# JuliaGraphics/Hikari.jl

Measured on AMD Instinct MI355X. Metric: Mrays/s, higher is better.
Workload: dtype f32

## Files before the change

### hikari.jl_amd/csrc/hk_ctx.cpp

```cpp
#include "hk_host.h"

thread_local std::string g_err;
SlabCache g_slabs;

namespace hk {
static thread_local const Knobs* tl_knobs = nullptr;
const char* knob(const char* name) {
    if (!tl_knobs) return nullptr;
    auto it = tl_knobs->kv.find(name);
    return it == tl_knobs->kv.end() ? nullptr : it->second.c_str();
}
static const char* const KNOB_NAMES[] = {
    "HK_BATCH_PATHS_M", "HK_BVH_LEAF", "HK_BVH_BINS", "HK_QNODES", "HK_DEBUG_ALLOC", "HK_DELTA_ADVANCE", "HK_DYNAMIC_SEGMENTS", "HK_GREY", "HK_GREY_COMPACT", "HK_GREY_FLAT", "HK_MAX_PATHS_M",
    "HK_MID_LISTS", "HK_MID_PASS_PATHS_M", "HK_NODE_CACHE", "HK_NVDB_DENSE_MB", "HK_OVERLAP", "HK_PIPELINE", "HK_PIPELINE_AFTER", "HK_PIPELINE_MAX_PATHS_M", "HK_PRESELECT",
    "HK_SELECT_MIN_IDLE", "HK_SHADOW_FEED_ROUNDS", "HK_SHADOW_TRACK_BATCH", "HK_SMALL_PASS", "HK_SMALL_PASS_WAVES", "HK_SOBOL_LO_GB", "HK_SOBOL_TABLE_ONLY",
    "HK_STATE_CACHE_GB", "HK_STATE_SLAB", "HK_TICKET_SHARE", "HK_TRACK_ADVANCE", "HK_TRACK_EXTRA_ADVANCE", "HK_TRACK_MIN_PENDING", "HK_TRACK_POOL", "HK_TRACK_REFILL_IDLE",
    "HK_WALK_POOL", "HK_WALK_REFILL_IDLE", "HK_WALK_SPLIT", "HK_WAVES_PER_CU", "HK_READBACK_PIN", "HK_DEFER_EXTERNAL", "HK_SELECT_POOL", "HK_SMALL_PASS_FUSED", "HK_SMALL_PASS_MERGED", "HK_OCC_SCALE", "HK_ESCAPED_UNROLL", "HK_SHADOW_FINAL", "HK_TRI_PACK", "HK_LEAN_RECORDS", "HK_VIEW_CACHE", "HK_MAJORANT_BLOCK_VOXELS", "HK_BVH_BUILD_SMALL", "HK_SHADE_LEAN", "HK_SHADE_PRESCAN", "HK_SHADE_PREFETCH"};
static bool known_knob(const char* name) {
    for (const char* k : KNOB_NAMES)
        if (std::strcmp(k, name) == 0) return true;
    return false;
}
}
KnobScope::KnobScope(const hk::Knobs* k) : prev(hk::tl_knobs) { hk::tl_knobs = k; }
KnobScope::~KnobScope() { hk::tl_knobs = prev; }

void quiesce(hk_ctx* c) {
    if (!c) return;
    (void)hipStreamSynchronize(c->stream);
    if (c->aux) (void)hipStreamSynchronize(c->aux);
    for (auto& l : c->lanes)
        if (l.stream) (void)hipStreamSynchronize(l.stream);
}
int join_lanes(hk_ctx* c) {
    if (!c) return HK_OK;
    if (int e = flush_pending(c)) return e;
    if (!c->lanes_dirty) return HK_OK;
    for (auto& l : c->lanes)
        if (l.done) HIP_TRY(hipStreamWaitEvent(c->stream, l.done, 0));
    c->lanes_dirty = false;
// ... 326 lines not shown
```

### hikari.jl_amd/csrc/hk_edit_host.h

```cpp
#pragma once
#include <algorithm>
#include <cmath>
#include <cstddef>
#include <cstring>
#include <vector>

#if defined(__HIPCC__)
#define HK_EDIT_HD __host__ __device__
#else
#define HK_EDIT_HD
#endif

HK_EDIT_HD inline double hk_box_area(const float lo[3], const float hi[3]) {
    if (!(lo[0] <= hi[0]) || !(lo[1] <= hi[1]) || !(lo[2] <= hi[2])) return 0.0;
    const double dx = (double)hi[0] - (double)lo[0], dy = (double)hi[1] - (double)lo[1], dz = (double)hi[2] - (double)lo[2];
    return 2.0 * ((dx * dy + dx * dz) + dy * dz);
}
HK_EDIT_HD inline double hk_node_cost(const float lo[2][3], const float hi[2][3], int c0, int c1) {
    const double w0 = c0 >= 0 ? 1.0 : (double)(((~c0) & 7) + 1), w1 = c1 >= 0 ? 1.0 : (double)(((~c1) & 7) + 1);
    return hk_box_area(lo[0], hi[0]) * w0 + hk_box_area(lo[1], hi[1]) * w1;
}
HK_EDIT_HD inline double hk_root_area(const float lo[2][3], const float hi[2][3]) {
    float l[3] = {INFINITY, INFINITY, INFINITY}, h[3] = {-INFINITY, -INFINITY, -INFINITY};
    for (int c = 0; c < 2; ++c) {
        if (!(lo[c][0] <= hi[c][0]) || !(lo[c][1] <= hi[c][1]) || !(lo[c][2] <= hi[c][2])) continue;
        for (int k = 0; k < 3; ++k) l[k] = lo[c][k] < l[k] ? lo[c][k] : l[k], h[k] = h[k] < hi[c][k] ? hi[c][k] : h[k];
    }
    return hk_box_area(l, h);
}

namespace hk {

template <class Material>
inline int materials_have_kind(const Material* m, size_t n, int kind) {
    for (size_t i = 0; i < n; ++i)
        if (m[i].kind == kind) return 1;
    return 0;
}
inline int single_material_kind(unsigned kinds_mask, int has_mix, int max_kinds) {
    if (has_mix || kinds_mask == 0u || (kinds_mask & (kinds_mask - 1u)) != 0u) return -1;
    int k = 0;
    while (!((kinds_mask >> k) & 1u)) ++k;
    return k < max_kinds ? k : -1;
}

inline bool stage_positions(const float* src, int first, int n, float* dst, int block, std::vector<float>& fresh) {
    fresh.clear();
    const int b0 = block > 0 ? first / block : 0;
    if (block > 0) {
        const int nb = (first + n - 1) / block - b0 + 1;
        fresh.resize(6 * (size_t)nb);
        for (int b = 0; b < nb; ++b)
            for (int k = 0; k < 3; ++k) fresh[6 * (size_t)b + k] = INFINITY, fresh[6 * (size_t)b + 3 + k] = -INFINITY;
    }
    bool finite = true;
    for (int i = 0; i < n; ++i) {
        const float* p = src + 9 * (size_t)i;
        std::memcpy(dst + 9 * (size_t)i, p, 36);
        for (int v = 0; v < 9; ++v) finite = finite && std::isfinite(p[v]);
        if (block > 0) {
            float* bb = fresh.data() + 6 * (size_t)((first + i) / block - b0);
            for (int v = 0; v < 9; ++v) {
                bb[v % 3] = std::min(bb[v % 3], p[v]);
                bb[3 + v % 3] = std::max(bb[3 + v % 3], p[v]);
            }
        }
    }
// ... 40 lines not shown
```

### hikari.jl_amd/csrc/hk_kernels.hip

```cpp
#include <hip/hip_runtime.h>
#include <type_traits>
#include <cstdlib>
#include <cstdio>

#include "hikari_mi355x.h"
#include "hk_device.h"
#include "hk_edit_host.h"
#include "hk_bvh_decide.h"

using namespace hkd;

namespace {

__device__ __forceinline__ int lane_id() { return (int)(threadIdx.x & 63); }

struct WaveQ {
    uint32_t* base;
    int count;
};
__device__ __forceinline__ int global_wave() {
    const int w = (int)(threadIdx.x >> 6), b = (int)blockIdx.x;
    if (blockDim.x == 1024 && (gridDim.x & 7) == 0) return ((((b >> 3) * 4 + (w >> 2)) * 8 + (b & 7)) << 2) + (w & 3);
    if (blockDim.x == 512 && (gridDim.x & 7) == 0) return ((((b >> 3) * 2 + (w >> 2)) * 8 + (b & 7)) << 2) + (w & 3);
    return b * (int)(blockDim.x >> 6) + w;
// ... 753 lines not shown
    HK_DBG_DECL
    HK_FOR_EACH_SEGMENT_FROM(gw, st, src) {
    const DPathGen g = gen_at(st, depth);
    const uint32_t seg = (uint32_t)gw * (uint32_t)st.wave_cap;
    const int n = *count_ptr(st, depth, Q_RAY, gw);
    WaveQ q_escaped = wq_open(st.escaped_q, st, gw);
    static_assert(!(SINGLE && MIX), "a scene with a MixMaterial is not a single-kind scene");
    int kind_count[HK_MAX_KINDS];
#pragma unroll
    for (int k = 0; k < HK_MAX_KINDS; ++k) kind_count[k] = 0;
    int one_count = 0;
    int cursor = 0;
    int state = LR_EMPTY;
    uint32_t slot = 0;
    LaneRay r;
    r.cur = r.pend = DONE;
    for (;;) {
        const unsigned long long run_m = __ballot(state == LR_ACTIVE && r.cur != DONE);
        if (run_m == 0ull || (64 - __popcll(run_m) >= MIN_IDLE && cursor < n)) {
            HK_DBG(8, state == LR_ACTIVE && r.cur == DONE);
            int kind = -1;
            uint32_t eflag = 0u;
            if (state == LR_ACTIVE && r.cur == DONE) {
                if (r.best.prim < 0)
                    kind = -2;
                else {
                    ++n_hits;
                    const DTriMeta hm = sc.meta[r.best.prim];
                    eflag = hm.arealight > 0 ? HK_MATQ_EMISSIVE : 0u;
                    int mat = sc.mis[hm.mi].material;
                    if (MIX && sc.materials[mat].kind == HK_MAT_MIX) {
                        float w = 1.0f - r.best.u - r.best.v;
                        mat = resolve_mix_material(sc, mat, r.o + r.d * r.best.t, -r.d, uv_at(sc, r.best.prim, w, r.best.u, r.best.v));
                    }
                    kind = SINGLE ? sc.single_kind : sc.materials[mat].kind;
                    if (MIX && kind == HK_MAT_MIX) kind = HK_MAT_FALLBACK;
                    stream_st(&st.hit[slot], make_float4(r.best.t, __int_as_float(r.best.prim), r.best.u, r.best.v));
                    stream_st(reinterpret_cast<uint32_t*>(st.mat_id) + slot, (uint32_t)(mat | (hm.arealight > 0 ? HK_MAT_EMISSIVE_BIT : 0)));
                }
                state = LR_EMPTY;
            }
            wq_push(q_escaped, slot, kind == -2);
            unsigned long long pending = __ballot(kind >= 0);
            if (SINGLE) {
                if (kind >= 0) stream_st(&st.mat_q[((size_t)sc.single_kind * st.n_waves + gw) * st.wave_cap + one_count + __popcll(pending & lt_mask)], slot | eflag);
                one_count += __popcll(pending);
                pending = 0ull;
            }
            while (pending) {
// ... 1545 lines not shown
    st4(&st.L[pmeta.y], ld4(&st.L[pmeta.y]) + fin);
}

template <int KIND>
struct ShadeWaves {
    static constexpr int value = (KIND == HK_MAT_COATED_DIFFUSE || KIND == HK_MAT_COATED_DIFFUSE_TRANSMISSION) ? 1 : (KIND == HK_MAT_MATTE ? HK_SHADE_WAVES_MATTE : HK_SHADE_WAVES);
};
#ifndef HK_SHADE_MIN_WAVES
#define HK_SHADE_MIN_WAVES 1
#endif
#define HK_SHADE_STASH 16
struct ShadeStage {
    uint32_t* entry;
    float4* hit;
    float4* ray_d;
    uint32_t* meta;
};
__device__ __forceinline__ void lds_fetch4(const uint32_t* src, uint32_t* lds_wave_base) {
    __builtin_amdgcn_global_load_lds((const __attribute__((address_space(1))) void*)src, (__attribute__((address_space(3))) void*)lds_wave_base, 4, 0, 0);
}
__device__ __forceinline__ void lds_fetch16(const float4* src, float4* lds_wave_base) {
    __builtin_amdgcn_global_load_lds((const __attribute__((address_space(1))) void*)src, (__attribute__((address_space(3))) void*)lds_wave_base, 16, 0, 0);
}
template <int KIND, bool SIMPLE, bool FT, bool PRE, bool LEAN = false>
__device__ __forceinline__ void shade_body(const DPathState& st, const DScene& sc, const DTables& T, const DFrame& fr, const DSobol& sob, int depth, int first_kind, DStats* stats, const SegTickets& src,
                                           uint32_t* __restrict__ elist,
                                           float* stash = nullptr,
                                           ShadeStage stage = ShadeStage{}) {
    static_assert(!LEAN || (KIND == HK_MAT_MATTE && HK_LAMBDA_BY_SLOT), "the lean body is Matte's");
    const int lane = lane_id();
    unsigned n_vertices = 0, n_lnodes = 0;
    unsigned nv_wave = 0;
    unsigned* const nl_stash = LEAN ? reinterpret_cast<unsigned*>(stash) + (HK_SHADE_STASH - 1) * 256 + threadIdx.x : nullptr;
    auto nl_flush = [&]() {
        if constexpr (LEAN) {
            if (n_lnodes) *nl_stash += n_lnodes;
            n_lnodes = 0;
        }
    };
    if constexpr (LEAN) *nl_stash = 0u;
    auto uni = [](int v) { return LEAN ? __builtin_amdgcn_readfirstlane(v) : v; };
    HK_FOR_EACH_SEGMENT_FROM(gw_v, st, src) {
    const int gw = uni(gw_v);
    const uint32_t* __restrict__ queue = st.mat_q + ((size_t)KIND * st.n_waves + gw) * st.wave_cap;
    const int n = uni(*count_ptr(st, depth, Q_MAT0 + KIND, gw));
    const DPathGen g = gen_at(st, depth), gn = st.gen[(depth + 1) & 1];
    const size_t seg = (size_t)gw * st.wave_cap;
    const bool ones = depth == 0 && fr.implicit_ones;
    WavePos q_shadow{0}, q_next{0};
    if (!first_kind) {
        q_shadow.count = uni(*count_ptr(st, depth, Q_SHADOW, gw));
        q_next.count = uni(*count_ptr(st, depth + 1, Q_RAY, gw));
    }
    int n_emit = 0;
    auto emit_pass = [&](int take) {
        __builtin_amdgcn_fence(__ATOMIC_SEQ_CST, "wavefront");
        if (lane < take) shade_emission<KIND == HK_MAT_MATTE, SIMPLE, LEAN>(st, g, ones, sc, T, elist[lane], n_lnodes, depth, seg);
        nl_flush();
        const int rest = n_emit - take;
        const uint32_t moved = lane < rest ? elist[64 + lane] : 0u;
        __builtin_amdgcn_fence(__ATOMIC_SEQ_CST, "wavefront");
        if (lane < rest) elist[lane] = moved;
        n_emit = rest;
    };
    const bool prescan = uni(st.shade_prescan) != 0;
    if (prescan) {
        for (int base = 0; base < n || n_emit > 0; base += 64) {
            if (base < n) {
                const int i = base + lane;
                const uint32_t cand = i < n ? queue[i] & ~HK_MATQ_EMISSIVE : 0u;
                const bool em = i < n && (st.mat_id[cand] & HK_MAT_EMISSIVE_BIT) != 0;
                const unsigned long long m = __ballot(em);
                if (em) elist[n_emit + __popcll(m & ((1ull << lane) - 1ull))] = cand;
                n_emit += __popcll(m);
                if (n_emit < 64 && base + 64 < n) continue;
            }
            emit_pass(n_emit < 64 ? n_emit : 64);
        }
    }
    const bool prefetch = LEAN && stage.entry != nullptr;
    const int wave0 = LEAN ? __builtin_amdgcn_readfirstlane((int)(threadIdx.x & ~63u)) : 0;
    if constexpr (LEAN) {
        if (prefetch && 64 + lane < n) lds_fetch4(&queue[64 + lane], stage.entry + 256 + wave0);
    }
    for (int base = 0; base < n; base += 64) {
        int i = base + lane;
        bool active = i < n;
        if constexpr (LEAN) {
            if (prefetch && i + 128 < n) lds_fetch4(&queue[i + 128], stage.entry + ((base >> 6) & 1) * 256 + wave0);
        }
        const bool staged = prefetch && base > 0;
        uint32_t slot = active ? queue[i] : 0u;
        {
            const bool em = !prescan && (slot & HK_MATQ_EMISSIVE) != 0u;
            slot &= ~HK_MATQ_EMISSIVE;
            const unsigned long long m = __ballot(em);
            if (m != 0ull) {
                if (em) elist[n_emit + __popcll(m & ((1ull << lane) - 1ull))] = slot;
                n_emit += __popcll(m);
                if (n_emit >= 64) emit_pass(64);
            }
        }
        bool push_shadow = false, push_ray = false;
        float4 H = make_float4(0, 0, 0, 0);
        Surface sf;
        v3 wo = mk3(0, 0, 1);
        DTriMeta meta{0u, 0u, 0u};
        S4 lambda = s4(0.0f), beta = s4(0.0f), r_u = s4(0.0f), kd_matte = s4(0.0f);
        uint32_t fl = 0, pslot = 0;
        int pdepth = 0, medium = -1;
        bool any_non_specular = false;
        SobolCtx sctx;
        using W = std::conditional_t<LEAN, float, S4>;
        auto stash_at = [&]() {
            int i = (int)threadIdx.x;
            asm volatile("" : "+v"(i));
            return stash + i;
        };
        const int base_dim = 6 + 7 * depth;
        float4 shO = make_float4(0, 0, 0, 0), shD = shO;
        S4 shLd = s4(0.0f);
        W shRu{}, shRl{};
        if constexpr (LEAN) nv_wave += (unsigned)(n - base < 64 ? n - base : 64);
        if (active) {
            if constexpr (!LEAN) ++n_vertices;
            float4 D;
            uint32_t meta_w = 0;
            if (LEAN && staged) {
                asm volatile("s_waitcnt vmcnt(0)" ::: "memory");
                const int t = (int)threadIdx.x;
                H = stage.hit[t], D = stage.ray_d[t], meta_w = stage.meta[t];
            } else {
                H = stream_ld(&st.hit[slot]);
                D = stream_ld(&g.ray_d[slot]);
                if constexpr (LEAN) meta_w = reinterpret_cast<const uint32_t*>(g.meta)[slot];
            }
            float4 O = ld_ray_o(st, g, slot, depth, seg);
            v3 ro = mk3(O.x, O.y, O.z), rd = mk3(D.x, D.y, D.z);
            float t_hit = H.x;
            int prim = __float_as_int(H.y);
            sf = surface_at(sc, prim, H.z, H.w, ro, rd, t_hit);
            wo = -rd;
            meta = tri_meta(sc, prim);
            if constexpr (LEAN) {
                pslot = meta_w & 0x3fffffffu;
                pdepth = depth;
                any_non_specular = (meta_w >> 31) != 0u;
            } else {
                const uint2 pmeta = ld_meta(st, g, slot, depth);
                fl = pmeta.x;
                pslot = pmeta.y;
// ... 52 lines not shown
                    asm volatile("" : "+v"(b2));
                    Surface s2 = surface_at(sc, prim, b2, H.w, ro, rd, t_hit);
                    sink = s2.pi.x + s2.n.y + s2.ns.z + s2.uv.x + s2.area;
                }
                if (HK_ABLATE == 6) {
                    v3 w2 = wo;
                    asm volatile("" : "+v"(w2.x), "+v"(w2.y), "+v"(w2.z));
                    float p2;
                    S4 f2 = eval_matte_kd(kd_matte, w2, sf.n, sf.ns, p2);
                    BSDFSample s2 = sample_matte_kd(sc, sc.materials[st.mat_id[slot] & ~HK_MAT_EMISSIVE_BIT], kd_matte, w2, sf.ns, TexCtx(sf.uv, meta.prim_index, H.z, H.w), mk2(H.z, H.w));
                    sink = f2.x + f2.w + p2 + s2.pdf + s2.wi.x + s2.f.y;
                }
                asm volatile("" : : "v"(sink));
            }
#endif

            if constexpr (LEAN) {
                float* sp = stash + threadIdx.x;
                sp[0 * 256] = sf.n.x, sp[1 * 256] = sf.n.y, sp[2 * 256] = sf.n.z;
                sp[3 * 256] = wo.x, sp[4 * 256] = wo.y, sp[5 * 256] = wo.z;
                sp[6 * 256] = kd_matte.x, sp[7 * 256] = kd_matte.y, sp[8 * 256] = kd_matte.z, sp[9 * 256] = kd_matte.w;
                sp[10 * 256] = beta.x, sp[11 * 256] = beta.y, sp[12 * 256] = beta.z, sp[13 * 256] = beta.w;
                sp[14 * 256] = __uint_as_float(meta_w);
                if (prefetch && i + 64 < n) {
                    asm volatile("s_waitcnt vmcnt(0)" ::: "memory");
                    const uint32_t ns = stage.entry[(((base >> 6) + 1) & 1) * 256 + (int)threadIdx.x] & ~HK_MATQ_EMISSIVE;
                    lds_fetch16(&st.hit[ns], stage.hit + wave0);
                    lds_fetch16(&g.ray_d[ns], stage.ray_d + wave0);
                    lds_fetch4(reinterpret_cast<const uint32_t*>(g.meta) + ns, stage.meta + wave0);
                }
            }
            if (sc.n_lights > 0) {
                const DMaterial& mat = sc.materials[st.mat_id[slot] & ~HK_MAT_EMISSIVE_BIT];
                float light_pmf;
                int light_idx;
                if constexpr (PRE) {
                    const uint2 pre = st.sel_light[slot];
                    light_idx = (int)pre.x;
                    light_pmf = __uint_as_float(pre.y);
                } else {
                    float light_select = sobol_1d<FT>(sctx, base_dim + 1);
                    light_idx = bvh_sample_light(sc, sf.pi, sf.ns, light_select, light_pmf, n_lnodes);
                }
                if (light_idx >= 1 && light_idx <= sc.n_lights && light_pmf > 0.0f) {
                    const DLight& sel = sc.lights[light_idx - 1];
                    v2 u_light = mk2(0.0f, 0.0f);
                    if (sel.kind >= HK_LIGHT_AMBIENT) u_light = sobol_2d<FT>(sctx, base_dim + 3);
// ... 139 lines not shown
                if (st.compact) nD.w = nrl.x;
                stream_st(&gn.ray_d[pn], nD);
                stream_st(&gn.beta[pn], nb);
                st_ru_rl(gn, pn, r_u, nrl, st.compact != 0);
                st_lambda(gn, pn, lambda);
                st_meta(st, gn, pn, nflags, pslot);
            }
        }
    }
    if (n_emit > 0) emit_pass(n_emit);
    if (lane == 0) {
        *count_ptr(st, depth, Q_SHADOW, gw) = q_shadow.count;
        *count_ptr(st, depth + 1, Q_RAY, gw) = q_next.count;
    }
    }
    if constexpr (LEAN) {
        n_vertices = lane == 0 ? nv_wave : 0u;
        n_lnodes = *nl_stash;
    }
    stats += global_wave();
    wave_add(&stats->vertices, n_vertices);
    wave_add(&stats->light_nodes, n_lnodes);
}
template <int KIND, bool SIMPLE = false, bool FT = false, bool PRE = false, bool LEAN = false>
__global__ void __attribute__((amdgpu_flat_work_group_size(256, 256), amdgpu_waves_per_eu(LEAN ? (FT ? HK_SHADE_WAVES_LEAN : HK_SHADE_WAVES_LEAN_HASH) : ShadeWaves<KIND>::value))) k_shade(DPathState st, DScene sc, DTables T, DFrame fr, DSobol sob, int depth, int first_kind, DStats* stats) {
    __shared__ uint32_t emit_list[4 * 128];
    SegTickets src = seg_open(st, ticket_ptr(st, depth, TK_SHADE0 + KIND), st.dynamic_segments != 0, depth, Q_MAT0 + KIND);
    if constexpr (LEAN) {
        src.pos = __builtin_amdgcn_readfirstlane(src.pos), src.k0 = __builtin_amdgcn_readfirstlane(src.k0);
        __shared__ float stash[HK_SHADE_STASH * 256];
        __shared__ uint32_t stage_entry[2 * 256];
        __shared__ float4 stage_hit[256];
        __shared__ float4 stage_ray_d[256];
        __shared__ uint32_t stage_meta[256];
        ShadeStage stage{};
        if (st.shade_prefetch) stage.entry = stage_entry, stage.hit = stage_hit, stage.ray_d = stage_ray_d, stage.meta = stage_meta;
        shade_body<KIND, SIMPLE, FT, PRE, true>(st, sc, T, fr, sob, depth, first_kind, stats, src, emit_list + (threadIdx.x >> 6) * 128, stash, stage);
    } else
        shade_body<KIND, SIMPLE, FT, PRE>(st, sc, T, fr, sob, depth, first_kind, stats, src, emit_list + (threadIdx.x >> 6) * 128);
}

template <class W> HKD W wone();
template <> HKD float wone<float>() { return 1.0f; }
template <> HKD S4 wone<S4>() { return s4(1.0f); }
HKD S4 wide(S4 v) { return v; }
HKD S4 wide(float v) { return s4(v); }
HKD bool is_black(float v) { return v == 0.0f; }
template <bool COMPACT>
HKD void shadow_contribute(const DPathState& st, uint32_t rec, S4 T_ray, S4 tr_u, S4 tr_l) {
    if (is_black(T_ray)) return;
    S4 w_u, w_l;
    ld_shadow_weights<COMPACT>(st, rec, w_u, w_l);
    S4 mis = w_u * tr_u + w_l * tr_l;
    float den = average(mis);
    if (den > 1e-10f) {
        S4 fin = ld4(&st.sh_Ld[rec]) * T_ray / den;
        if (!is_black(fin)) {
            const uint32_t pslot = st.sh_slot[rec];
            st4(&st.L[pslot], ld4(&st.L[pslot]) + fin);
        }
// ... 2180 lines not shown
```

### hikari.jl_amd/csrc/hk_launch_impl.h

```cpp
#pragma once
#include "hk_launch.h"

namespace hk {

template <bool V>
using bool_c = std::bool_constant<V>;
template <int V>
using int_c = std::integral_constant<int, V>;
template <class F>
static void with_bool(bool b, F&& f) {
    if (b) f(bool_c<true>{});
    else f(bool_c<false>{});
}
template <int V0, int... Vs, class F>
static void with_int(int v, F&& f) {
    if constexpr (sizeof...(Vs) == 0) f(int_c<V0>{});
    else if (v == V0) f(int_c<V0>{});
    else with_int<Vs...>(v, f);
}

#ifndef HK_OCC_SCALE_DEFAULT
#define HK_OCC_SCALE_DEFAULT 1.0f
#endif
static inline int grid_for(int n, int block, int cap) {
// ... 73 lines not shown
#endif
#ifndef HK_SHADOW_BLOCK16
#define HK_SHADOW_BLOCK16 768
#endif
#ifndef HK_SHADOW_NC32
#define HK_SHADOW_NC32 0
#endif
#ifndef HK_TRACE_SINGLE_KIND
#define HK_TRACE_SINGLE_KIND 1
#endif
#ifndef HK_TRACE_NC32
#define HK_TRACE_NC32 128
#endif
template <int B16, int NC16, int NC32, class F>
static void lean_dispatch(const DScene& sc, const DFrame& fr, F&& launch) {
    with_bool(fr.count_nodes != 0, [&](auto COUNT) {
        with_bool(node_cache_on(), [&](auto CACHE) {
            constexpr bool cache = decltype(CACHE)::value;
            if (sc.bvh_depth <= 16) launch(COUNT, int_c<16>{}, int_c<cache ? B16 : HK_TRACE_BLOCK>{}, int_c<cache ? NC16 : 0>{}, bool_c<false>{});
            else with_bool(sc.qnodes != nullptr, [&](auto QN) { launch(COUNT, int_c<HK_LDS_STACK>{}, int_c<HK_TRACE_BLOCK>{}, int_c<cache ? NC32 : 0>{}, QN); });
        });
    });
}
void launch_trace(hipStream_t s, int n_cu, const DPathState& st, const DScene& sc, const DTables& T, const DFrame& fr, int depth, DStats* stats) {
    if (lean_scene(sc)) {
        const int flush = sc.has_mix ? 0 : (HK_TRACE_SINGLE_KIND && sc.single_kind >= 0 ? 2 : 1);
        lean_dispatch<1024, 1536, HK_TRACE_NC32>(sc, fr, [&](auto COUNT, auto STACK, auto BLOCK, auto NC, auto QN) {
            constexpr int block = decltype(BLOCK)::value;
            constexpr bool count = decltype(COUNT)::value;
            with_int<2, 1, 0>(flush, [&](auto FLUSH) {
                constexpr int f = count ? 0 : decltype(FLUSH)::value;
                launch_resident<k_trace_lean<count, decltype(STACK)::value, block, decltype(NC)::value, decltype(QN)::value, f == 0, f == 2>>(s, n_cu, st, block, 8, sc, depth, stats);
            });
        });
        return;
    }
    with_bool(fr.count_nodes != 0, [&](auto COUNT) { launch_resident<k_trace<decltype(COUNT)::value>>(s, n_cu, st, HK_TRACE_BLOCK, 8, sc, T, fr, depth, stats); });
}
template <bool C, int MM>
static void launch_walk_split(hipStream_t s, int n_cu, const DPathState& st, const DScene& sc, const DFrame& fr, int depth, DStats* stats) {
    const int cb = clamp_blocks(cached_blocks<k_walk_cast<C, MM, 16>>(HK_TRACE_BLOCK, n_cu, 8), st);
    const int tb = clamp_blocks(cached_blocks<k_walk_track<MM>>(256, n_cu, 8), st);
    for (int round = 0; round < HK_WALK_ROUNDS; ++round) {
        hipLaunchKernelGGL((k_walk_cast<C, MM, 16>), dim3(cb), dim3(HK_TRACE_BLOCK), 0, s, st, sc, depth, round, stats, sc.media);
        hipLaunchKernelGGL((k_walk_track<MM>), dim3(tb), dim3(256), 0, s, st, sc, depth, round, fr.walk_tune, stats, sc.media);
    }
}
bool grey_compact_ok(const DScene& sc) {
    if (!knob_on("HK_GREY_COMPACT")) return false;
// ... 86 lines not shown
    hipLaunchKernelGGL(k_detect_camera_medium, dim3(1), dim3(64), 0, s, st, sc, x, y, z, stats);
}
void launch_escaped(hipStream_t s, int n_cu, const DPathState& st, const DScene& sc, const DTables& T, const DFrame& fr, int depth) {
    with_bool(knob_int("HK_ESCAPED_UNROLL", 1) != 2, [&](auto ONE) { launch_resident<k_escaped<decltype(ONE)::value ? 1 : 2>>(s, n_cu, st, 256, 8, sc, T, depth, fr.implicit_ones); });
}
bool preselect_lights(const DScene& sc, const DPathState& st) {
    return sc.n_media == 0 && sc.num_bvh_lights >= HK_PRESELECT_MIN && st.sel_light != nullptr && knob_on("HK_PRESELECT");
}
void launch_light_select(hipStream_t s, int n_cu, const DPathState& st, const DScene& sc, const DTables& T, const DFrame& fr, const DSobol& sob, int depth, uint32_t kinds_mask, DStats* stats) {
    const int min_idle = knob_int_in("HK_SELECT_MIN_IDLE", 1, 64, HK_SELECT_MIN_IDLE);
    const bool pool = knob_on("HK_SELECT_POOL");
    with_bool(sobol_tables_cover(sob, depth), [&](auto FT) {
        constexpr bool ft = decltype(FT)::value;
        if (pool) launch_resident<k_light_select_pool<ft>>(s, n_cu, st, HK_SELECT_BLOCK, 8, sc, T, fr, sob, depth, kinds_mask, stats);
        else launch_resident<k_light_select<ft>>(s, n_cu, st, 256, 8, sc, T, fr, sob, depth, kinds_mask, min_idle, stats);
    });
}
void launch_shade(hipStream_t s, int n_cu, int kind, const DPathState& st, const DScene& sc, const DTables& T, const DFrame& fr, const DSobol& sob, int depth, int first_kind, DStats* stats) {
    auto shade = [&](auto KIND, auto SIMPLE, auto FT, auto PRE) {
        launch_resident<k_shade<decltype(KIND)::value, decltype(SIMPLE)::value, decltype(FT)::value, decltype(PRE)::value>>(s, n_cu, st, 256, 8, sc, T, fr, sob, depth, first_kind, stats);
    };
    const bool ft = sobol_tables_cover(sob, depth);
    if (kind == HK_MAT_MATTE && sc.simple_lights && lean_scene(sc) && st.compact && st.meta32 && st.sh_final && !preselect_lights(sc, st) && knob_on("HK_SHADE_LEAN")) {
        with_bool(ft, [&](auto FT) { launch_resident<k_shade<HK_MAT_MATTE, true, decltype(FT)::value, false, true>>(s, n_cu, st, 256, 8, sc, T, fr, sob, depth, first_kind, stats); });
        return;
    }
    const bool light_kind = kind == HK_MAT_MATTE || kind == HK_MAT_MIRROR || kind == HK_MAT_GLASS || kind == HK_MAT_CONDUCTOR;
    if (light_kind && preselect_lights(sc, st))
        with_int<HK_MAT_MATTE, HK_MAT_MIRROR, HK_MAT_GLASS, HK_MAT_CONDUCTOR>(kind, [&](auto KIND) { with_bool(ft, [&](auto FT) { shade(KIND, bool_c<false>{}, FT, bool_c<true>{}); }); });
    else if (kind == HK_MAT_MATTE && sc.simple_lights)
        with_bool(ft, [&](auto FT) { shade(int_c<HK_MAT_MATTE>{}, bool_c<true>{}, FT, bool_c<false>{}); });
    else if (light_kind && ft)
        with_int<HK_MAT_MATTE, HK_MAT_MIRROR, HK_MAT_GLASS, HK_MAT_CONDUCTOR>(kind, [&](auto KIND) { shade(KIND, bool_c<false>{}, bool_c<true>{}, bool_c<false>{}); });
    else
        with_int<HK_MAT_MATTE, HK_MAT_MIRROR, HK_MAT_GLASS, HK_MAT_CONDUCTOR, HK_MAT_COATED_DIFFUSE, HK_MAT_THIN_DIELECTRIC, HK_MAT_DIFFUSE_TRANSMISSION, HK_MAT_COATED_DIFFUSE_TRANSMISSION,
                 HK_MAT_COATED_CONDUCTOR, HK_MAT_FALLBACK>(kind, [&](auto KIND) { shade(KIND, bool_c<false>{}, bool_c<false>{}, bool_c<false>{}); });
}
#ifndef HK_SMALL_PASS_NC
#define HK_SMALL_PASS_NC 1536
#endif
static int small_pass_class(const DScene& sc, uint32_t kinds_mask) {
    const int mode = knob_int("HK_SMALL_PASS_FUSED", 2);
    if (mode == 0) return 0;
    if (!(lean_scene(sc) && sc.bvh_depth <= HK_LDS_STACK && node_cache_on())) return 0;
    if (kinds_mask == (1u << HK_MAT_MATTE) && sc.simple_lights && !sc.has_escape_lights && sc.bvh_depth <= 16 && sc.num_bvh_lights < HK_PRESELECT_MIN) return 1;
    const uint32_t light_kinds = (1u << HK_MAT_MATTE) | (1u << HK_MAT_MIRROR) | (1u << HK_MAT_GLASS) | (1u << HK_MAT_CONDUCTOR);
    return (mode >= 2 && kinds_mask != 0 && (kinds_mask & ~light_kinds) == 0) ? 2 : 0;
// ... 166 lines not shown
```

### hikari.jl_amd/csrc/hk_render.cpp

```cpp
#include "hk_host.h"

namespace {
float gaussian_1d(float x, float sigma) { return std::exp(-(x * x) / (2.0f * (sigma * sigma))); }
float mitchell_1d(float x, float B, float C) {
    x = std::fabs(x);
    if (x <= 1.0f) return ((12.0f - 9.0f * B - 6.0f * C) * (x * x * x) + (-18.0f + 12.0f * B + 6.0f * C) * (x * x) + (6.0f - 2.0f * B)) / 6.0f;
    if (x <= 2.0f) return ((-B - 6.0f * C) * (x * x * x) + (6.0f * B + 30.0f * C) * (x * x) + (-12.0f * B - 48.0f * C) * x + (8.0f * B + 24.0f * C)) / 6.0f;
    return 0.0f;
}
float sinc1(float x) {
    x = std::fabs(x);
    if (x < 1e-5f) return 1.0f;
    x *= 3.14159265358979323846f;
    return std::sin(x) / x;
}
float wsinc(float x, float r, float tau) {
    x = std::fabs(x);
    if (x > r) return 0.0f;
    return sinc1(x) * sinc1(x / tau);
}
float filter_eval(const hk_integrator_params& p, float ex, float ey, float x, float y) {
    float rx = p.filter_radius[0], ry = p.filter_radius[1];
    switch (p.filter_type) {
        case HK_FILTER_BOX: return (std::fabs(x) <= rx && std::fabs(y) <= ry) ? 1.0f : 0.0f;
// ... 192 lines not shown
}
int ensure_state(hk_integrator* I, int capacity, const PassTraits& t, hipStream_t users) {
    const bool media = t.media, open_scene = t.open_scene, small_scene = t.small_scene, grey_compact = t.grey_compact, fusable = t.fusable, lean = t.lean;
    const int n_cu = I->ctx->n_cu;
    long mid_paths = 48L << 20;
    if (const char* e = hk::knob("HK_MID_PASS_PATHS_M")) mid_paths = std::atol(e) >= 0 ? std::atol(e) << 20 : mid_paths;
    const bool mid = !media && !open_scene && small_scene && (long)capacity <= mid_paths;
    I->mid_pass = mid;
    const long cap_per_cu = media ? 96 : ((open_scene || mid) ? 48 : 192);
    long W_want = ((long)(capacity + 63) / 64) / 16;
    if (W_want < 4L * n_cu) W_want = 4L * n_cu;
    if (W_want > cap_per_cu * n_cu) W_want = cap_per_cu * n_cu;
    I->ctx->waves_per_cu = hk::knob_int_in("HK_WAVES_PER_CU", 1, INT_MAX, 0);
    if (I->ctx->waves_per_cu > 0) W_want = (long)I->ctx->waves_per_cu * n_cu;
    W_want = (W_want + 3) / 4 * 4;
    I->st.dynamic_segments = (media || (!open_scene && !mid)) ? 1 : 0;
    I->st.dynamic_segments = hk::knob_int("HK_DYNAMIC_SEGMENTS", I->st.dynamic_segments) ? 1 : 0;
    I->st.compact = media ? (grey_compact ? 1 : 0) : 1;
    I->st.sh_final = (lean && hk::knob_on("HK_SHADOW_FINAL")) ? 1 : 0;
    I->st.meta32 = (lean && hk::knob_on("HK_LEAN_RECORDS")) ? 1 : 0;
    I->st.const_origin = 0;
    I->st.shade_prescan = hk::knob_int("HK_SHADE_PRESCAN", 0) != 0 ? 1 : 0;
    I->st.shade_prefetch = hk::knob_on("HK_SHADE_PREFETCH") ? 1 : 0;
    I->st.ticket_share = hk::knob_int("HK_TICKET_SHARE", 1) ? 1 : 0;
    {
        const bool small_on = hk::knob_on("HK_SMALL_PASS");
        const bool small = W_want <= 4L * n_cu && small_on && hk::knob("HK_DYNAMIC_SEGMENTS") == nullptr;
        I->st.small_pass = small ? 1 : 0;
        if (mid && I->st.dynamic_segments == 0 && small_on && !hk::knob_int("HK_MID_LISTS", 0))
            I->st.small_pass = 1;
        if (small) {
            I->st.dynamic_segments = 0;
            const int w = hk::knob_int_in("HK_SMALL_PASS_WAVES", 1, INT_MAX, 0);
            long per_cu = w > 0 ? w : (users ? (media ? 4 : 8) : (((open_scene && !media) || fusable) ? 8 : 16));
            const long chunks = ((long)capacity + 63) / 64;
            while (per_cu > 4 && per_cu * n_cu > chunks) per_cu /= 2;
            if (I->ctx->waves_per_cu <= 0) W_want = (per_cu * n_cu + 3) / 4 * 4;
        }
    }
    const bool want_split = media && hk::walk_split_mode();
    const bool want_cam = !media && !users && hk::knob_on("HK_VIEW_CACHE");
    if (I->st_capacity >= capacity && I->st_depth >= I->p.max_depth && I->st.n_waves == (int)W_want && I->st_media == (media ? 1 : 0) && (!want_split || I->st.wq_a != nullptr) &&
        (!want_cam || I->cam_gen.ray_d != nullptr || I->cam_unfit))
        return HK_OK;
    I->view_key.clear();
    if (users) HIP_TRY(hipStreamSynchronize(users));
// ... 500 lines not shown
```

### hikari.jl_amd/csrc/hk_test_api.cpp

```cpp
#include "hk_host.h"

namespace {
struct Tmp {
    std::vector<void*> ptrs;
    ~Tmp() {
        for (void* p : ptrs) (void)hipFree(p);
    }
    template <class T>
    T* up(const T* src, size_t n) {
        void* p = nullptr;
        if (hipMalloc(&p, (n ? n : 1) * sizeof(T)) != hipSuccess) return nullptr;
        ptrs.push_back(p);
        if (src && n) (void)hipMemcpy(p, src, n * sizeof(T), hipMemcpyHostToDevice);
        return (T*)p;
    }
};
}

extern "C" int32_t hk_trace_closest(hk_ctx* c, hk_scene* sc, int32_t n, const float* o3, const float* d3, const float* tmax, float* out_t, int32_t* out_prim,
                                    float* out_uv2) {
    if (!c || !sc || n < 0) return fail(HK_ERR_INVALID, "bad argument");
    HIP_TRY(hipSetDevice(c->device));
    KnobScope knobs(&c->knobs);
    Tmp t;
// ... 148 lines not shown
    HIP_TRY(hipMemcpy(out_t, ot, (size_t)n * 4, hipMemcpyDeviceToHost));
    HIP_TRY(hipMemcpy(out_prim, op, (size_t)n * 4, hipMemcpyDeviceToHost));
    HIP_TRY(hipMemcpy(out_uv2, ouv, 2 * (size_t)n * 4, hipMemcpyDeviceToHost));
    return HK_OK;
}

extern "C" int32_t hk_test_medium_bricks(hk_scene* s, int32_t idx, int32_t* dims, float* out) {
    if (!s || !dims) return fail(HK_ERR_INVALID, "hk_test_medium_bricks: null argument");
    if (idx < 0 || idx >= (int)s->h_media.size()) return fail(HK_ERR_INVALID, "hk_test_medium_bricks: medium index out of range");
    const DMedium& d = s->h_media[idx].d;
    for (int k = 0; k < 3; ++k) dims[k] = d.nv_bricks ? d.nvb_dim[k] : 0;
    if (!d.nv_bricks || !out) return HK_OK;
    hk_ctx* c = s->ctx;
    HIP_TRY(hipSetDevice(c->device));
    KnobScope knobs(&c->knobs);
    if (int e = join_lanes(c)) return e;
    HIP_TRY(hipStreamSynchronize(c->stream));
    HIP_TRY(hipMemcpy(out, d.nv_bricks, (size_t)d.nvb_dim[0] * d.nvb_dim[1] * d.nvb_dim[2] * 729 * sizeof(float), hipMemcpyDeviceToHost));
    return HK_OK;
}

extern "C" int32_t hk_test_queue_counts(hk_integrator* I, int32_t depth, int32_t kind, int32_t* n_segments, int32_t* counts, int32_t* flagged) {
    if (!I || !n_segments) return fail(HK_ERR_INVALID, "hk_test_queue_counts: null argument");
    if (kind < 0 || kind >= HK_MAX_KINDS || depth < 0 || depth >= I->st_depth + 2) return fail(HK_ERR_INVALID, "hk_test_queue_counts: kind or depth out of range");
    if (!I->st.counters) return fail(HK_ERR_INVALID, "hk_test_queue_counts: no pass has been rendered");
    *n_segments = I->st.n_waves;
    if (!counts) return HK_OK;
    hk_ctx* c = I->ctx;
    HIP_TRY(hipSetDevice(c->device));
    KnobScope knobs(&c->knobs);
    if (int e = join_lanes(c)) return e;
    HIP_TRY(hipStreamSynchronize(c->stream));
    HIP_TRY(hipMemcpy(counts, I->st.counters + (size_t)(depth * Q_COUNT + Q_MAT0 + kind) * I->st.n_waves, (size_t)I->st.n_waves * sizeof(int), hipMemcpyDeviceToHost));
    if (!flagged) return HK_OK;
    const size_t Q = (size_t)I->st.n_waves * I->st.wave_cap;
    std::vector<uint32_t> q(Q);
    HIP_TRY(hipMemcpy(q.data(), I->st.mat_q + (size_t)kind * Q, Q * sizeof(uint32_t), hipMemcpyDeviceToHost));
    for (int w = 0; w < I->st.n_waves; ++w) {
        int n = 0;
        for (int i = 0; i < counts[w] && i < I->st.wave_cap; ++i) n += (q[(size_t)w * I->st.wave_cap + i] & HK_MATQ_EMISSIVE) != 0u;
        flagged[w] = n;
    }
    return HK_OK;
}
```

### hikari.jl_amd/csrc/hk_types.h

```cpp
#pragma once
#include <hip/hip_runtime.h>
#include <stdint.h>
#include <cstdlib>

namespace hk {
const char* knob(const char* name);
inline bool knob_on(const char* name) {
    const char* e = knob(name);
    return !(e && std::atoi(e) == 0);
}
inline int knob_int(const char* name, int dflt) {
    const char* e = knob(name);
    return e ? std::atoi(e) : dflt;
}
inline int knob_int_in(const char* name, int lo, int hi, int dflt) {
    const int v = knob_int(name, dflt);
    return v >= lo && v <= hi ? v : dflt;
}
}

#define HK_TICKET_COLS 16
#define HK_TICKET_WAYS 64
#define HK_TICKET_STRIDE 64
#define HK_MAX_KINDS 11
#ifndef HK_LDS_STACK
#define HK_LDS_STACK 32
#endif
#define HK_TRACE_BLOCK 256

struct DNode {
    float4 a;
    float4 b;
    float4 c;
    int c0, c1;
    int pad0, pad1;
};

#define HK_MAT_EMISSIVE_BIT 0x40000000
#define HK_MATQ_EMISSIVE 0x80000000u
#define HK_TRI_OPAQUE 1u

struct DSpectrumParam {
    float4 coef;
    float rgba[4];
    int tex;
    int pad[3];
};

struct DMaterial {
    int kind, flags;
    int i[4];
    int spectrum[2];
    DSpectrumParam rgb[4];
    float f[8];
    int ftex[8];
    uint32_t mix_key[4];
};

struct DTexture {
    const float* data;
    int width, height, channels, pad;
// ... 316 lines not shown
    uint32_t* wq_a;
    uint32_t* wq_b;
    int* wq_ctl;
    uint32_t* escaped_q;
    uint32_t* medium_q;
    uint32_t* scatter_q;
    int* initial_medium;
    uint32_t* mat_q;
    int* counters;
    int* tickets;
    int ticket_rows;
    int* seg_list;
    int* seg_list_n;
    int dynamic_segments;
    int small_pass;
    int ticket_share;
    int compact;
    int meta32, const_origin;
    int sh_final;
    DPathGen gen_cam;
    int view_cache;
    int shade_prescan;
    int shade_prefetch;
};

struct DStats {
    unsigned long long rays_closest, rays_shadow, nodes, tris, hits, vertices, collisions, light_nodes, sh_nodes, sh_tris;
    unsigned long long nvdb_collisions, sh_nvdb_collisions;
    unsigned long long sh_collisions, dda_steps, sh_dda_steps, scatter_vertices, sc_light_nodes;
#ifdef HK_DEBUG_UTIL
    unsigned long long dbg[32];
#endif
};

struct DFrame {
    int width, height, tiles_x, tiles_y;
    int x0, y0, x1, y1;
    int n_pixels_padded;
    int samples_in_pass;
    uint32_t s_mul;
    int s_shr;
    int first_sample, sample_stride;
    int max_depth;
    int regularize;
    float max_component_value;
    int count_nodes;
// ... 32 lines not shown
```

Before: 11180.

## Walk ray slots directly in lean Matte shade instead of material queue

```diff
diff --git a/hikari.jl_amd/csrc/hk_ctx.cpp b/hikari.jl_amd/csrc/hk_ctx.cpp
--- a/hikari.jl_amd/csrc/hk_ctx.cpp
+++ b/hikari.jl_amd/csrc/hk_ctx.cpp
@@ -15,7 +15,7 @@
     "HK_MID_LISTS", "HK_MID_PASS_PATHS_M", "HK_NODE_CACHE", "HK_NVDB_DENSE_MB", "HK_OVERLAP", "HK_PIPELINE", "HK_PIPELINE_AFTER", "HK_PIPELINE_MAX_PATHS_M", "HK_PRESELECT",
     "HK_SELECT_MIN_IDLE", "HK_SHADOW_FEED_ROUNDS", "HK_SHADOW_TRACK_BATCH", "HK_SMALL_PASS", "HK_SMALL_PASS_WAVES", "HK_SOBOL_LO_GB", "HK_SOBOL_TABLE_ONLY",
     "HK_STATE_CACHE_GB", "HK_STATE_SLAB", "HK_TICKET_SHARE", "HK_TRACK_ADVANCE", "HK_TRACK_EXTRA_ADVANCE", "HK_TRACK_MIN_PENDING", "HK_TRACK_POOL", "HK_TRACK_REFILL_IDLE",
-    "HK_WALK_POOL", "HK_WALK_REFILL_IDLE", "HK_WALK_SPLIT", "HK_WAVES_PER_CU", "HK_READBACK_PIN", "HK_DEFER_EXTERNAL", "HK_SELECT_POOL", "HK_SMALL_PASS_FUSED", "HK_SMALL_PASS_MERGED", "HK_OCC_SCALE", "HK_ESCAPED_UNROLL", "HK_SHADOW_FINAL", "HK_TRI_PACK", "HK_LEAN_RECORDS", "HK_VIEW_CACHE", "HK_MAJORANT_BLOCK_VOXELS", "HK_BVH_BUILD_SMALL", "HK_SHADE_LEAN", "HK_SHADE_PRESCAN", "HK_SHADE_PREFETCH"};
+    "HK_WALK_POOL", "HK_WALK_REFILL_IDLE", "HK_WALK_SPLIT", "HK_WAVES_PER_CU", "HK_READBACK_PIN", "HK_DEFER_EXTERNAL", "HK_SELECT_POOL", "HK_SMALL_PASS_FUSED", "HK_SMALL_PASS_MERGED", "HK_OCC_SCALE", "HK_ESCAPED_UNROLL", "HK_SHADOW_FINAL", "HK_TRI_PACK", "HK_LEAN_RECORDS", "HK_VIEW_CACHE", "HK_MAJORANT_BLOCK_VOXELS", "HK_BVH_BUILD_SMALL", "HK_SHADE_LEAN", "HK_SHADE_PRESCAN", "HK_SHADE_PREFETCH", "HK_SHADE_SLOT_WALK"};
 static bool known_knob(const char* name) {
     for (const char* k : KNOB_NAMES)
         if (std::strcmp(k, name) == 0) return true;
diff --git a/hikari.jl_amd/csrc/hk_edit_host.h b/hikari.jl_amd/csrc/hk_edit_host.h
--- a/hikari.jl_amd/csrc/hk_edit_host.h
+++ b/hikari.jl_amd/csrc/hk_edit_host.h
@@ -43,6 +43,8 @@
     while (!((kinds_mask >> k) & 1u)) ++k;
     return k < max_kinds ? k : -1;
 }
+inline bool shade_slot_walk_wanted(bool slot_walk_knob, bool prescan, bool lean_knob) { return slot_walk_knob && !prescan && lean_knob; }
+inline bool shade_slot_walk_launch(int wanted, int single_kind, int kind, bool single_flush) { return wanted != 0 && single_kind >= 0 && single_kind == kind && single_flush; }
 
 inline bool stage_positions(const float* src, int first, int n, float* dst, int block, std::vector<float>& fresh) {
     fresh.clear();
diff --git a/hikari.jl_amd/csrc/hk_kernels.hip b/hikari.jl_amd/csrc/hk_kernels.hip
--- a/hikari.jl_amd/csrc/hk_kernels.hip
+++ b/hikari.jl_amd/csrc/hk_kernels.hip
@@ -799,9 +799,10 @@
             int kind = -1;
             uint32_t eflag = 0u;
             if (state == LR_ACTIVE && r.cur == DONE) {
-                if (r.best.prim < 0)
+                if (r.best.prim < 0) {
                     kind = -2;
-                else {
+                    if constexpr (SINGLE) stream_st(reinterpret_cast<uint32_t*>(st.mat_id) + slot, HK_MAT_ESCAPED);
+                } else {
                     ++n_hits;
                     const DTriMeta hm = sc.meta[r.best.prim];
                     eflag = hm.arealight > 0 ? HK_MATQ_EMISSIVE : 0u;
@@ -2393,12 +2394,13 @@
 __device__ __forceinline__ void lds_fetch16(const float4* src, float4* lds_wave_base) {
     __builtin_amdgcn_global_load_lds((const __attribute__((address_space(1))) void*)src, (__attribute__((address_space(3))) void*)lds_wave_base, 16, 0, 0);
 }
-template <int KIND, bool SIMPLE, bool FT, bool PRE, bool LEAN = false>
+template <int KIND, bool SIMPLE, bool FT, bool PRE, bool LEAN = false, bool SLOTS = false>
 __device__ __forceinline__ void shade_body(const DPathState& st, const DScene& sc, const DTables& T, const DFrame& fr, const DSobol& sob, int depth, int first_kind, DStats* stats, const SegTickets& src,
                                            uint32_t* __restrict__ elist,
                                            float* stash = nullptr,
                                            ShadeStage stage = ShadeStage{}) {
     static_assert(!LEAN || (KIND == HK_MAT_MATTE && HK_LAMBDA_BY_SLOT), "the lean body is Matte's");
+    static_assert(!SLOTS || LEAN, "the slot walk is the lean body's");
     const int lane = lane_id();
     unsigned n_vertices = 0, n_lnodes = 0;
     unsigned nv_wave = 0;
@@ -2414,7 +2416,7 @@
     HK_FOR_EACH_SEGMENT_FROM(gw_v, st, src) {
     const int gw = uni(gw_v);
     const uint32_t* __restrict__ queue = st.mat_q + ((size_t)KIND * st.n_waves + gw) * st.wave_cap;
-    const int n = uni(*count_ptr(st, depth, Q_MAT0 + KIND, gw));
+    const int n = uni(*count_ptr(st, depth, SLOTS ? Q_RAY : Q_MAT0 + KIND, gw));
     const DPathGen g = gen_at(st, depth), gn = st.gen[(depth + 1) & 1];
     const size_t seg = (size_t)gw * st.wave_cap;
     const bool ones = depth == 0 && fr.implicit_ones;
@@ -2434,7 +2436,7 @@
         if (lane < rest) elist[lane] = moved;
         n_emit = rest;
     };
-    const bool prescan = uni(st.shade_prescan) != 0;
+    const bool prescan = !SLOTS && uni(st.shade_prescan) != 0;
     if (prescan) {
         for (int base = 0; base < n || n_emit > 0; base += 64) {
             if (base < n) {
@@ -2451,20 +2453,36 @@
     }
     const bool prefetch = LEAN && stage.entry != nullptr;
     const int wave0 = LEAN ? __builtin_amdgcn_readfirstlane((int)(threadIdx.x & ~63u)) : 0;
-    if constexpr (LEAN) {
+    if constexpr (LEAN && !SLOTS) {
         if (prefetch && 64 + lane < n) lds_fetch4(&queue[64 + lane], stage.entry + 256 + wave0);
     }
     for (int base = 0; base < n; base += 64) {
         int i = base + lane;
         bool active = i < n;
-        if constexpr (LEAN) {
+        if constexpr (LEAN && !SLOTS) {
             if (prefetch && i + 128 < n) lds_fetch4(&queue[i + 128], stage.entry + ((base >> 6) & 1) * 256 + wave0);
         }
         const bool staged = prefetch && base > 0;
-        uint32_t slot = active ? queue[i] : 0u;
+        float4 H_staged = make_float4(0, 0, 0, 0), D_staged = H_staged;
+        uint32_t meta_staged = 0;
+        uint32_t slot;
+        bool em_slot = false;
+        if constexpr (SLOTS) {
+            slot = (uint32_t)seg + (uint32_t)i;
+            uint32_t mat_w = HK_MAT_ESCAPED;
+            if (staged) {
+                asm volatile("s_waitcnt vmcnt(0)" ::: "memory");
+                const uint32_t w = stage.entry[(int)threadIdx.x];
+                if (active) mat_w = w;
+            } else if (active)
+                mat_w = reinterpret_cast<const uint32_t*>(st.mat_id)[slot];
+            active = mat_w != HK_MAT_ESCAPED;
+            em_slot = active && (mat_w & HK_MAT_EMISSIVE_BIT) != 0u;
+        } else
+            slot = active ? queue[i] : 0u;
         {
-            const bool em = !prescan && (slot & HK_MATQ_EMISSIVE) != 0u;
-            slot &= ~HK_MATQ_EMISSIVE;
+            const bool em = SLOTS ? em_slot : !prescan && (slot & HK_MATQ_EMISSIVE) != 0u;
+            if constexpr (!SLOTS) slot &= ~HK_MATQ_EMISSIVE;
             const unsigned long long m = __ballot(em);
             if (m != 0ull) {
                 if (em) elist[n_emit + __popcll(m & ((1ull << lane) - 1ull))] = slot;
@@ -2472,8 +2490,23 @@
                 if (n_emit >= 64) emit_pass(64);
             }
         }
+        if constexpr (SLOTS) {
+            if (staged) {
+                const int t = (int)threadIdx.x;
+                H_staged = stage.hit[t], D_staged = stage.ray_d[t], meta_staged = stage.meta[t];
+                asm volatile("" : "+v"(H_staged.x), "+v"(H_staged.y), "+v"(H_staged.z), "+v"(H_staged.w), "+v"(D_staged.x), "+v"(D_staged.y), "+v"(D_staged.z), "+v"(D_staged.w), "+v"(meta_staged) : : "memory");
+            }
+            if (prefetch && i + 64 < n) {
+                const uint32_t ns = slot + 64u;
+                lds_fetch4(reinterpret_cast<const uint32_t*>(st.mat_id) + ns, stage.entry + wave0);
+                lds_fetch16(&st.hit[ns], stage.hit + wave0);
+                lds_fetch16(&g.ray_d[ns], stage.ray_d + wave0);
+                lds_fetch4(reinterpret_cast<const uint32_t*>(g.meta) + ns, stage.meta + wave0);
+            }
+        }
         bool push_shadow = false, push_ray = false;
         float4 H = make_float4(0, 0, 0, 0);
+        if constexpr (SLOTS) H = H_staged;
         Surface sf;
         v3 wo = mk3(0, 0, 1);
         DTriMeta meta{0u, 0u, 0u};
@@ -2492,12 +2525,15 @@
         float4 shO = make_float4(0, 0, 0, 0), shD = shO;
         S4 shLd = s4(0.0f);
         W shRu{}, shRl{};
-        if constexpr (LEAN) nv_wave += (unsigned)(n - base < 64 ? n - base : 64);
+        if constexpr (SLOTS) nv_wave += (unsigned)__popcll(__ballot(active));
+        else if constexpr (LEAN) nv_wave += (unsigned)(n - base < 64 ? n - base : 64);
         if (active) {
             if constexpr (!LEAN) ++n_vertices;
             float4 D;
             uint32_t meta_w = 0;
-            if (LEAN && staged) {
+            if (SLOTS && staged)
+                D = D_staged, meta_w = meta_staged;
+            else if (LEAN && staged) {
                 asm volatile("s_waitcnt vmcnt(0)" ::: "memory");
                 const int t = (int)threadIdx.x;
                 H = stage.hit[t], D = stage.ray_d[t], meta_w = stage.meta[t];
@@ -2596,7 +2632,7 @@
                 sp[6 * 256] = kd_matte.x, sp[7 * 256] = kd_matte.y, sp[8 * 256] = kd_matte.z, sp[9 * 256] = kd_matte.w;
                 sp[10 * 256] = beta.x, sp[11 * 256] = beta.y, sp[12 * 256] = beta.z, sp[13 * 256] = beta.w;
                 sp[14 * 256] = __uint_as_float(meta_w);
-                if (prefetch && i + 64 < n) {
+                if (!SLOTS && prefetch && i + 64 < n) {
                     asm volatile("s_waitcnt vmcnt(0)" ::: "memory");
                     const uint32_t ns = stage.entry[(((base >> 6) + 1) & 1) * 256 + (int)threadIdx.x] & ~HK_MATQ_EMISSIVE;
                     lds_fetch16(&st.hit[ns], stage.hit + wave0);
@@ -2782,7 +2818,7 @@
     wave_add(&stats->vertices, n_vertices);
     wave_add(&stats->light_nodes, n_lnodes);
 }
-template <int KIND, bool SIMPLE = false, bool FT = false, bool PRE = false, bool LEAN = false>
+template <int KIND, bool SIMPLE = false, bool FT = false, bool PRE = false, bool LEAN = false, bool SLOTS = false>
 __global__ void __attribute__((amdgpu_flat_work_group_size(256, 256), amdgpu_waves_per_eu(LEAN ? (FT ? HK_SHADE_WAVES_LEAN : HK_SHADE_WAVES_LEAN_HASH) : ShadeWaves<KIND>::value))) k_shade(DPathState st, DScene sc, DTables T, DFrame fr, DSobol sob, int depth, int first_kind, DStats* stats) {
     __shared__ uint32_t emit_list[4 * 128];
     SegTickets src = seg_open(st, ticket_ptr(st, depth, TK_SHADE0 + KIND), st.dynamic_segments != 0, depth, Q_MAT0 + KIND);
@@ -2795,7 +2831,7 @@
         __shared__ uint32_t stage_meta[256];
         ShadeStage stage{};
         if (st.shade_prefetch) stage.entry = stage_entry, stage.hit = stage_hit, stage.ray_d = stage_ray_d, stage.meta = stage_meta;
-        shade_body<KIND, SIMPLE, FT, PRE, true>(st, sc, T, fr, sob, depth, first_kind, stats, src, emit_list + (threadIdx.x >> 6) * 128, stash, stage);
+        shade_body<KIND, SIMPLE, FT, PRE, true, SLOTS>(st, sc, T, fr, sob, depth, first_kind, stats, src, emit_list + (threadIdx.x >> 6) * 128, stash, stage);
     } else
         shade_body<KIND, SIMPLE, FT, PRE>(st, sc, T, fr, sob, depth, first_kind, stats, src, emit_list + (threadIdx.x >> 6) * 128);
 }
diff --git a/hikari.jl_amd/csrc/hk_launch_impl.h b/hikari.jl_amd/csrc/hk_launch_impl.h
--- a/hikari.jl_amd/csrc/hk_launch_impl.h
+++ b/hikari.jl_amd/csrc/hk_launch_impl.h
@@ -119,9 +119,10 @@
         });
     });
 }
+static int lean_flush(const DScene& sc, const DFrame& fr) { return (sc.has_mix || fr.count_nodes) ? 0 : (HK_TRACE_SINGLE_KIND && sc.single_kind >= 0 ? 2 : 1); }
 void launch_trace(hipStream_t s, int n_cu, const DPathState& st, const DScene& sc, const DTables& T, const DFrame& fr, int depth, DStats* stats) {
     if (lean_scene(sc)) {
-        const int flush = sc.has_mix ? 0 : (HK_TRACE_SINGLE_KIND && sc.single_kind >= 0 ? 2 : 1);
+        const int flush = lean_flush(sc, fr);
         lean_dispatch<1024, 1536, HK_TRACE_NC32>(sc, fr, [&](auto COUNT, auto STACK, auto BLOCK, auto NC, auto QN) {
             constexpr int block = decltype(BLOCK)::value;
             constexpr bool count = decltype(COUNT)::value;
@@ -254,7 +255,12 @@
     };
     const bool ft = sobol_tables_cover(sob, depth);
     if (kind == HK_MAT_MATTE && sc.simple_lights && lean_scene(sc) && st.compact && st.meta32 && st.sh_final && !preselect_lights(sc, st) && knob_on("HK_SHADE_LEAN")) {
-        with_bool(ft, [&](auto FT) { launch_resident<k_shade<HK_MAT_MATTE, true, decltype(FT)::value, false, true>>(s, n_cu, st, 256, 8, sc, T, fr, sob, depth, first_kind, stats); });
+        const bool slots = shade_slot_walk_launch(st.shade_slot_walk, sc.single_kind, kind, lean_flush(sc, fr) == 2);
+        with_bool(ft, [&](auto FT) {
+            with_bool(slots, [&](auto SLOTS) {
+                launch_resident<k_shade<HK_MAT_MATTE, true, decltype(FT)::value, false, true, decltype(SLOTS)::value>>(s, n_cu, st, 256, 8, sc, T, fr, sob, depth, first_kind, stats);
+            });
+        });
         return;
     }
     const bool light_kind = kind == HK_MAT_MATTE || kind == HK_MAT_MIRROR || kind == HK_MAT_GLASS || kind == HK_MAT_CONDUCTOR;
diff --git a/hikari.jl_amd/csrc/hk_render.cpp b/hikari.jl_amd/csrc/hk_render.cpp
--- a/hikari.jl_amd/csrc/hk_render.cpp
+++ b/hikari.jl_amd/csrc/hk_render.cpp
@@ -238,6 +238,7 @@
     I->st.const_origin = 0;
     I->st.shade_prescan = hk::knob_int("HK_SHADE_PRESCAN", 0) != 0 ? 1 : 0;
     I->st.shade_prefetch = hk::knob_on("HK_SHADE_PREFETCH") ? 1 : 0;
+    I->st.shade_slot_walk = hk::shade_slot_walk_wanted(hk::knob_on("HK_SHADE_SLOT_WALK"), I->st.shade_prescan != 0, hk::knob_on("HK_SHADE_LEAN")) ? 1 : 0;
     I->st.ticket_share = hk::knob_int("HK_TICKET_SHARE", 1) ? 1 : 0;
     {
         const bool small_on = hk::knob_on("HK_SMALL_PASS");
diff --git a/hikari.jl_amd/csrc/hk_test_api.cpp b/hikari.jl_amd/csrc/hk_test_api.cpp
--- a/hikari.jl_amd/csrc/hk_test_api.cpp
+++ b/hikari.jl_amd/csrc/hk_test_api.cpp
@@ -194,7 +194,9 @@
 
 extern "C" int32_t hk_test_queue_counts(hk_integrator* I, int32_t depth, int32_t kind, int32_t* n_segments, int32_t* counts, int32_t* flagged) {
     if (!I || !n_segments) return fail(HK_ERR_INVALID, "hk_test_queue_counts: null argument");
-    if (kind < 0 || kind >= HK_MAX_KINDS || depth < 0 || depth >= I->st_depth + 2) return fail(HK_ERR_INVALID, "hk_test_queue_counts: kind or depth out of range");
+    if (kind < -2 || kind >= HK_MAX_KINDS || depth < 0 || depth >= I->st_depth + 2) return fail(HK_ERR_INVALID, "hk_test_queue_counts: kind or depth out of range");
+    if (kind < 0 && flagged) return fail(HK_ERR_INVALID, "hk_test_queue_counts: only a kind's queue has flagged entries");
+    const int queue = kind == -1 ? Q_RAY : (kind == -2 ? Q_ESCAPED : Q_MAT0 + kind);
     if (!I->st.counters) return fail(HK_ERR_INVALID, "hk_test_queue_counts: no pass has been rendered");
     *n_segments = I->st.n_waves;
     if (!counts) return HK_OK;
@@ -203,7 +205,7 @@
     KnobScope knobs(&c->knobs);
     if (int e = join_lanes(c)) return e;
     HIP_TRY(hipStreamSynchronize(c->stream));
-    HIP_TRY(hipMemcpy(counts, I->st.counters + (size_t)(depth * Q_COUNT + Q_MAT0 + kind) * I->st.n_waves, (size_t)I->st.n_waves * sizeof(int), hipMemcpyDeviceToHost));
+    HIP_TRY(hipMemcpy(counts, I->st.counters + (size_t)(depth * Q_COUNT + queue) * I->st.n_waves, (size_t)I->st.n_waves * sizeof(int), hipMemcpyDeviceToHost));
     if (!flagged) return HK_OK;
     const size_t Q = (size_t)I->st.n_waves * I->st.wave_cap;
     std::vector<uint32_t> q(Q);
diff --git a/hikari.jl_amd/csrc/hk_types.h b/hikari.jl_amd/csrc/hk_types.h
--- a/hikari.jl_amd/csrc/hk_types.h
+++ b/hikari.jl_amd/csrc/hk_types.h
@@ -37,6 +37,7 @@
 };
 
 #define HK_MAT_EMISSIVE_BIT 0x40000000
+#define HK_MAT_ESCAPED 0xffffffffu
 #define HK_MATQ_EMISSIVE 0x80000000u
 #define HK_TRI_OPAQUE 1u
 
@@ -399,6 +400,7 @@
     int view_cache;
     int shade_prescan;
     int shade_prefetch;
+    int shade_slot_walk;
 };
 
 struct DStats {
```

Result: faster. 11360, median of 6 (+1.6%).
